# tl32rodan/DCVC

Hardware: AMD Instinct MI355X
Metric: encode+decode fps @1920x1080 per GPU; bpp bit-exact + PSNR Δ<1e-4 dB vs ref (higher is better)
Workload: dtype f32 (convs on split-fp16 f16x3 MFMA, fp32 accumulation); 1 GPU; C3 DCVC-DC RGB 1920x1080 (pad 1920x1088) IP=32 write mode; gop=32, precision=split, q_index=0, stream_part=8, parallelism=sequence-sharded x1, 3 GOP lane(s) per GPU, lanes=3, step=one frame on each of 3 lane(s)

## Files before the change

dcvc_amd/csrc/hip/sdc.hip:

```cpp
#include "common.h"
#include "split.h"

namespace {

constexpr int kNW = 8, kNT = kNW * 64;
constexpr int TH = 8, TW = 16;
constexpr int HW_ = TW + 2, NPH = (TH + 2) * HW_;
constexpr int HR = 192;

struct DP {
  const float *x;
  int H, W, xcs, xco;
  float *y;
  int ycs, yco;
  const uint16_t *w;
  int wbytes;
  const float *b1, *wdw, *bdw, *b2, *ba;
  float slope;
  int tiles_x, ntiles;
  int *ovf;
};

template <int CIN, int COUT, bool ADAPT>
struct DG {
  static constexpr int KCI = (CIN + 31) / 32;
  static constexpr int NTI = (CIN + 15) / 16, NTO = (COUT + 15) / 16;
  static constexpr int CI16 = NTI * 16, CO16 = NTO * 16;
  static constexpr int W1 = KCI * CI16 * 32, W2 = KCI * CO16 * 32, WA = ADAPT ? KCI * CO16 * 32 : 0;
  static constexpr int NWH = 2 * (W1 + W2 + WA);
  static constexpr int XI = KCI * HR * 32;
  static constexpr int DI = KCI * TH * TW * 32;
  static constexpr size_t OX = 0, OD = OX + (size_t)2 * XI * 2, OW = OD + (size_t)2 * DI * 2;
  static constexpr size_t OC = OW + (size_t)NWH * 2;
  static constexpr int NC = CIN * 11 + 2 * COUT;
  static constexpr size_t LDS = OC + (size_t)NC * 4;
  static constexpr int QP = CIN / 8;
  static constexpr int PP = (NPH * QP + kNT - 1) / kNT;
};

__device__ __forceinline__ float lrelu(float v, float s) { return fmaxf(v, v * s); }

template <int CIN, int COUT, bool ADAPT>
__global__ void __launch_bounds__(kNT) sdc_kernel(DP p) {
  SplitRange rg(p.ovf);
  typedef DG<CIN, COUT, ADAPT> G_;
  constexpr int KCI = G_::KCI, NTI = G_::NTI, NTO = G_::NTO, CO16 = G_::CO16, CI16 = G_::CI16;
  constexpr int XI = G_::XI, DI = G_::DI, QP = G_::QP, PP = G_::PP;
  extern __shared__ __align__(16) unsigned char smem[];
  uint16_t *Xh = reinterpret_cast<uint16_t *>(smem + G_::OX), *Xl = Xh + XI;
  uint16_t *Dh = reinterpret_cast<uint16_t *>(smem + G_::OD), *Dl = Dh + DI;
  uint16_t *W1h = reinterpret_cast<uint16_t *>(smem + G_::OW), *W1l = W1h + G_::W1;
  uint16_t *W2h = W1l + G_::W1, *W2l = W2h + G_::W2;
  uint16_t *WAh = W2l + G_::W2, *WAl = WAh + G_::WA;
  float *Lb1 = reinterpret_cast<float *>(smem + G_::OC), *Lbdw = Lb1 + CIN, *Lwdw = Lbdw + CIN;
  float *Lb2 = Lwdw + 9 * CIN, *Lba = Lb2 + COUT;
  auto t1p = [&](int r, int c) -> float * {
    return reinterpret_cast<float *>((c & 16) ? Xl : Xh) + (((c >> 5) * HR + r) * 16 + (c & 15));
  };

  const int tid = threadIdx.x;
  const int wave = tid >> 6, lane = tid & 63;
  const int col = lane & 15, hi = lane >> 4;
  const int G = gridDim.x;
  int g = blockIdx.x;
  if ((G & 7) == 0) g = (g & 7) * (G >> 3) + (g >> 3);
  if (g >= p.ntiles) return;

  {
    const __amdgpu_buffer_rsrc_t wr =
        __builtin_amdgcn_make_buffer_rsrc(const_cast<uint16_t *>(p.w), (short)0, p.wbytes, 0x00020000);
    constexpr int ND = G_::NWH * 2 / 1024;
    for (int i = wave; i < ND; i += kNW)
      __builtin_amdgcn_raw_ptr_buffer_load_lds(wr, (__attribute__((address_space(3))) void *)(W1h + i * 512), 16,
                                               i * 1024 + lane * 16, 0, 0, 0);
    for (int i = tid; i < G_::NC; i += kNT) {
      float v;
      if (i < CIN) v = p.b1[i];
      else if (i < 2 * CIN) v = p.bdw[i - CIN];
      else if (i < 11 * CIN) v = p.wdw[i - 2 * CIN];
      else if (i < 11 * CIN + COUT) v = p.b2[i - 11 * CIN];
      else v = ADAPT ? p.ba[i - 11 * CIN - COUT] : 0.f;
      Lb1[i] = v;
    }
  }

  const __amdgpu_buffer_rsrc_t xr = __builtin_amdgcn_make_buffer_rsrc(
      const_cast<float *>(p.x), (short)0,
      (int)((int64_t)p.H * p.W * p.xcs * 4 < 0x7fff0000 ? (int64_t)p.H * p.W * p.xcs * 4 : 0x7fff0000), 0x00020000);
  int pyx[PP], prel[PP], pofs[PP];
#pragma unroll
  for (int u = 0; u < PP; ++u) {
    const int it = tid + u * kNT;
    pyx[u] = -1;
    prel[u] = 0;
    pofs[u] = 0;
    if (it < NPH * QP) {
      const int pix = it / QP, q = it - pix * QP;
      const int hy = pix / HW_, hx = pix - hy * HW_;
      pyx[u] = (hy << 8) | hx;
      prel[u] = ((hy - 1) * p.W + (hx - 1)) * p.xcs + p.xco + q * 8;
      pofs[u] = swz((q >> 2) * HR + pix, q & 3);
    }
  }
  float pf[PP][8];
  auto prefetch = [&](int t) {
    const int oy0 = (t / p.tiles_x) * TH, ox0 = (t % p.tiles_x) * TW;
    const int base = oy0 * p.W + ox0;
#pragma unroll
    for (int u = 0; u < PP; ++u) {
      const int gy = oy0 - 1 + (pyx[u] >> 8), gx = ox0 - 1 + (pyx[u] & 255);
      const bool in = pyx[u] >= 0 && (unsigned)gy < (unsigned)p.H && (unsigned)gx < (unsigned)p.W;
      const int o = in ? (base * p.xcs + prel[u]) * 4 : 0x7fffffe0;
      const f32x4 a = __builtin_bit_cast(f32x4, __builtin_amdgcn_raw_buffer_load_b128(xr, o, 0, 0));
      const f32x4 b = __builtin_bit_cast(f32x4, __builtin_amdgcn_raw_buffer_load_b128(xr, o + 16, 0, 0));
#pragma unroll
      for (int j = 0; j < 4; ++j) {
        pf[u][j] = a[j];
        pf[u][4 + j] = b[j];
      }
    }
  };
  prefetch(g);

  auto zero_pad = [&]() {
    if constexpr (CIN % 32 != 0) {
      constexpr int PADQ = KCI * 4 - QP;
      for (int it = tid; it < HR * PADQ; it += kNT) {
        const int row = it / PADQ, q = QP + it % PADQ;
        const int o = swz((q >> 2) * HR + row, q & 3);
        *reinterpret_cast<u32x4_t *>(Xh + o) = u32x4_t{0u, 0u, 0u, 0u};
        *reinterpret_cast<u32x4_t *>(Xl + o) = u32x4_t{0u, 0u, 0u, 0u};
      }
    }
  };

  wait_vm_lgkm();
  for (int t = g; t < p.ntiles; t += G) {
    const int oy0 = (t / p.tiles_x) * TH, ox0 = (t % p.tiles_x) * TW;
    raw_barrier();
#pragma unroll
    for (int u = 0; u < PP; ++u) {
      u32x4_t h, l;
      rg.add8(pf[u]);
      split8(pf[u], h, l);
      if (pyx[u] >= 0) {
        *reinterpret_cast<u32x4_t *>(Xh + pofs[u]) = h;
        *reinterpret_cast<u32x4_t *>(Xl + pofs[u]) = l;
      }
    }
    zero_pad();
    wait_lgkm();
    raw_barrier();
    if (t + G < p.ntiles) prefetch(t + G);

    f32x4 idn[NTO];
    if constexpr (ADAPT) {
      f32x4 am[NTO], ac[NTO];
#pragma unroll
      for (int j = 0; j < NTO; ++j) {
        am[j] = f32x4{0.f, 0.f, 0.f, 0.f};
        ac[j] = f32x4{0.f, 0.f, 0.f, 0.f};
      }
      const int hr = (wave + 1) * HW_ + 1 + col;
#pragma unroll
      for (int kc = 0; kc < KCI; ++kc) {
        const int ob = swz(kc * HR + hr, hi);
        const f16x8 bh = *reinterpret_cast<const f16x8 *>(Xh + ob), bl = *reinterpret_cast<const f16x8 *>(Xl + ob);
#pragma unroll
        for (int j = 0; j < NTO; ++j) {
          const int oa = swz(kc * CO16 + j * 16 + col, hi);
          const f16x8 ah = *reinterpret_cast<const f16x8 *>(WAh + oa), al = *reinterpret_cast<const f16x8 *>(WAl + oa);
          am[j] = __builtin_amdgcn_mfma_f32_16x16x32_f16(ah, bh, am[j], 0, 0, 0);
          ac[j] = __builtin_amdgcn_mfma_f32_16x16x32_f16(ah, bl, ac[j], 0, 0, 0);
          ac[j] = __builtin_amdgcn_mfma_f32_16x16x32_f16(al, bh, ac[j], 0, 0, 0);
        }
      }
#pragma unroll
      for (int j = 0; j < NTO; ++j) {
        const int n = j * 16 + hi * 4;
#pragma unroll
        for (int e = 0; e < 4; ++e) idn[j][e] = (am[j][e] + ac[j][e] * kLoInv) + Lba[n + e < COUT ? n + e : 0];
      }
      wait_lgkm();
      raw_barrier();
    }

    for (int ht = wave; ht < HR / 16; ht += kNW) {
      f32x4 tm[NTI], tc[NTI];
#pragma unroll
      for (int j = 0; j < NTI; ++j) {
        tm[j] = f32x4{0.f, 0.f, 0.f, 0.f};
        tc[j] = f32x4{0.f, 0.f, 0.f, 0.f};
      }
      const int r = ht * 16 + col;
#pragma unroll
      for (int kc = 0; kc < KCI; ++kc) {
        const int ob = swz(kc * HR + r, hi);
        const f16x8 bh = *reinterpret_cast<const f16x8 *>(Xh + ob), bl = *reinterpret_cast<const f16x8 *>(Xl + ob);
#pragma unroll
        for (int j = 0; j < NTI; ++j) {
          const int oa = swz(kc * CI16 + j * 16 + col, hi);
          const f16x8 ah = *reinterpret_cast<const f16x8 *>(W1h + oa), al = *reinterpret_cast<const f16x8 *>(W1l + oa);
          tm[j] = __builtin_amdgcn_mfma_f32_16x16x32_f16(ah, bh, tm[j], 0, 0, 0);
          tc[j] = __builtin_amdgcn_mfma_f32_16x16x32_f16(ah, bl, tc[j], 0, 0, 0);
          tc[j] = __builtin_amdgcn_mfma_f32_16x16x32_f16(al, bh, tc[j], 0, 0, 0);
        }
      }
      const int hy = r / HW_, hx = r - hy * HW_;
      const int gy = oy0 - 1 + hy, gx = ox0 - 1 + hx;
      const bool inside = r < NPH && (unsigned)gy < (unsigned)p.H && (unsigned)gx < (unsigned)p.W;
      wave_lds_sync();
#pragma unroll
      for (int j = 0; j < NTI; ++j) {
        const int n = j * 16 + hi * 4;
        if (n >= CIN) continue;
        f32x4 v;
#pragma unroll
        for (int e = 0; e < 4; ++e) v[e] = inside ? lrelu((tm[j][e] + tc[j][e] * kLoInv) + Lb1[n + e], p.slope) : 0.f;
        *reinterpret_cast<f32x4 *>(t1p(r, n)) = v;
      }
    }
    wait_lgkm();
    raw_barrier();

    {
      constexpr int CG = CIN / 4;
      constexpr int R = kNT / (CG * TW) >= 4 ? 4 : kNT / (CG * TW) >= 2 ? 2 : 1;
      constexpr int RR = TH / R;
      static_assert(CG * TW * R <= kNT && TH % R == 0, "P2 tasks");
      if (tid < CG * TW * R) {
        const int cg = tid % CG, rest = tid / CG;
        const int ix = rest % TW, y0 = (rest / TW) * RR;
        const int c = cg * 4;
        f32x4 wv[9];
#pragma unroll
        for (int k = 0; k < 9; ++k) wv[k] = *reinterpret_cast<const f32x4 *>(Lwdw + k * CIN + c);
        const float4 bd = *reinterpret_cast<const float4 *>(Lbdw + c);
        f32x4 win[3][3];
#pragma unroll
        for (int r = 0; r < 2; ++r)
#pragma unroll
          for (int dx = 0; dx < 3; ++dx)
            win[r][dx] = *reinterpret_cast<const f32x4 *>(t1p((y0 + r) * HW_ + ix + dx, c));
#pragma unroll
        for (int i = 0; i < RR; ++i) {
#pragma unroll
          for (int dx = 0; dx < 3; ++dx)
            win[(i + 2) % 3][dx] = *reinterpret_cast<const f32x4 *>(t1p((y0 + i + 2) * HW_ + ix + dx, c));
          f32x4 a = f32x4{0.f, 0.f, 0.f, 0.f};
#pragma unroll
          for (int dy = 0; dy < 3; ++dy)
#pragma unroll
            for (int dx = 0; dx < 3; ++dx)
#pragma unroll
              for (int e = 0; e < 4; ++e) a[e] = __builtin_fmaf(wv[dy * 3 + dx][e], win[(i + dy) % 3][dx][e], a[e]);
          float v[4];
          v[0] = a[0] + bd.x;
          v[1] = a[1] + bd.y;
          v[2] = a[2] + bd.z;
          v[3] = a[3] + bd.w;
          rg.add4(v);
          const auto h01 = __builtin_amdgcn_cvt_pkrtz(v[0], v[1]);
          const auto h23 = __builtin_amdgcn_cvt_pkrtz(v[2], v[3]);
          const uint32_t l01 = pk(split_lo(v[0], (float)h01[0]), split_lo(v[1], (float)h01[1]));
          const uint32_t l23 = pk(split_lo(v[2], (float)h23[0]), split_lo(v[3], (float)h23[1]));
          const int px = (y0 + i) * TW + ix;
          const int o = swz((c >> 5) * (TH * TW) + px, (c & 31) >> 3) + (c & 7);
          typedef unsigned int u32x2_t __attribute__((ext_vector_type(2)));
          *reinterpret_cast<u32x2_t *>(Dh + o) = u32x2_t{__builtin_bit_cast(uint32_t, h01), __builtin_bit_cast(uint32_t, h23)};
          *reinterpret_cast<u32x2_t *>(Dl + o) = u32x2_t{l01, l23};
        }
      }
      if constexpr (CIN % 32 != 0) {
        constexpr int PADQ = KCI * 4 - CIN / 8;
        for (int it = tid; it < TH * TW * PADQ; it += kNT) {
          const int px = it / PADQ, q = CIN / 8 + it % PADQ;
          const int o = swz((q >> 2) * (TH * TW) + px, q & 3);
          *reinterpret_cast<u32x4_t *>(Dh + o) = u32x4_t{0u, 0u, 0u, 0u};
          *reinterpret_cast<u32x4_t *>(Dl + o) = u32x4_t{0u, 0u, 0u, 0u};
        }
      }
    }
    wait_lgkm();
    raw_barrier();

    {
      f32x4 cm[NTO], cc[NTO];
#pragma unroll
      for (int j = 0; j < NTO; ++j) {
        cm[j] = f32x4{0.f, 0.f, 0.f, 0.f};
        cc[j] = f32x4{0.f, 0.f, 0.f, 0.f};
      }
#pragma unroll
      for (int kc = 0; kc < KCI; ++kc) {
        const int ob = swz(kc * (TH * TW) + wave * TW + col, hi);
        const f16x8 bh = *reinterpret_cast<const f16x8 *>(Dh + ob), bl = *reinterpret_cast<const f16x8 *>(Dl + ob);
#pragma unroll
        for (int j = 0; j < NTO; ++j) {
          const int oa = swz(kc * CO16 + j * 16 + col, hi);
          const f16x8 ah = *reinterpret_cast<const f16x8 *>(W2h + oa), al = *reinterpret_cast<const f16x8 *>(W2l + oa);
          cm[j] = __builtin_amdgcn_mfma_f32_16x16x32_f16(ah, bh, cm[j], 0, 0, 0);
          cc[j] = __builtin_amdgcn_mfma_f32_16x16x32_f16(ah, bl, cc[j], 0, 0, 0);
          cc[j] = __builtin_amdgcn_mfma_f32_16x16x32_f16(al, bh, cc[j], 0, 0, 0);
        }
      }
      const int gy = oy0 + wave, gx = ox0 + col;
      if (gy < p.H && gx < p.W) {
        const int64_t pix = (int64_t)gy * p.W + gx;
#pragma unroll
        for (int j = 0; j < NTO; ++j) {
          const int n = j * 16 + hi * 4;
          if (n >= COUT) continue;
          f32x4 id;
          if constexpr (ADAPT) id = idn[j];
          else id = *reinterpret_cast<const f32x4 *>(p.x + pix * p.xcs + p.xco + n);
          f32x4 v;
#pragma unroll
          for (int e = 0; e < 4; ++e) v[e] = ((cm[j][e] + cc[j][e] * kLoInv) + Lb2[n + e]) + id[e];
          *reinterpret_cast<f32x4 *>(p.y + pix * p.ycs + p.yco + n) = v;
        }
      }
    }
  }
  wait_vm_lgkm();
}

int g_cus = 0;

template <int CIN, int COUT, bool ADAPT>
int run(DP p, hipStream_t st) {
  typedef DG<CIN, COUT, ADAPT> G_;
  static_assert(G_::LDS <= 160 * 1024, "LDS");
  static_assert(G_::NWH * 2 % 1024 == 0, "weight images in whole 1-KiB pieces");
  p.tiles_x = (p.W + TW - 1) / TW;
  const int64_t nt = (int64_t)p.tiles_x * ((p.H + TH - 1) / TH);
  if (nt <= 0) return DCVC_HIP_OK;
  p.ntiles = (int)nt;
  if (g_cus <= 0) {
    int dev = 0;
    hipDeviceProp_t prop;
    if (hipGetDevice(&dev) != hipSuccess || hipGetDeviceProperties(&prop, dev) != hipSuccess) return DCVC_HIP_ELAUNCH;
    g_cus = prop.multiProcessorCount;
  }
  int G = g_cus;
  if (G > p.ntiles) G = p.ntiles;
  auto kern = sdc_kernel<CIN, COUT, ADAPT>;
  dcvc_note_kernel("sdc_kernel<%d, %d, %s>@%lld", CIN, COUT, bname(ADAPT), (long long)G * kNT);
  dcvc_ensure_lds(reinterpret_cast<const void *>(kern), (int)G_::LDS);
  hipLaunchKernelGGL(kern, dim3((unsigned)G), dim3(kNT), G_::LDS, st, p);
  DCVC_LAUNCH_CHECK();
  return DCVC_HIP_OK;
}

bool supported(int cin, int cout, bool adapt) {
  return (cin == 64 && cout == 48 && adapt) || (cin == 48 && cout == 32 && adapt) ||
         (cin == 64 && cout == 64 && !adapt) || (cin == 32 && cout == 64 && adapt) ||
         (cin == 48 && cout == 48 && !adapt) || (cin == 32 && cout == 32 && !adapt);
}

}

extern "C" int64_t dcvc_dc_pack_weights(const float *w1, const float *w2, const float *wa, int cin, int cout,
                                        void *out) {
  if (!w1 || !w2 || cin <= 0 || cout <= 0) return DCVC_HIP_EINVAL;
  if (out && (!host_split_range_ok(w1, (int64_t)cin * cin) || !host_split_range_ok(w2, (int64_t)cout * cin) ||
              (wa && !host_split_range_ok(wa, (int64_t)cout * cin))))
    return DCVC_HIP_EINVAL;
  const int kci = (cin + 31) / 32, ci16 = (cin + 15) / 16 * 16, co16 = (cout + 15) / 16 * 16;
  const int64_t n1 = (int64_t)kci * ci16 * 32, n2 = (int64_t)kci * co16 * 32, na = wa ? n2 : 0;
  const int64_t total = 2 * (n1 + n2 + na);
  if (!out) return total;
  uint16_t *o = reinterpret_cast<uint16_t *>(out);
  auto at = [](int row, int k) {
    const int x = (0x1320 >> (((row >> 2) & 3) << 2)) & 3;
    return (int64_t)row * 32 + ((((k >> 3) ^ x) & 3) << 3) + (k & 7);
  };
  auto put = [&](uint16_t *img, int64_t n, const float *w, int rows, int rows16) {
    for (int kc = 0; kc < kci; ++kc)
      for (int r = 0; r < rows16; ++r)
        for (int k = 0; k < 32; ++k) {
          const int ch = kc * 32 + k;
          const float v = (r < rows && ch < cin) ? w[(int64_t)r * cin + ch] : 0.f;
          const int64_t q = at(kc * rows16 + r, k);
          host_split(v, img[q], img[n + q]);
        }
  };
  put(o, n1, w1, cin, ci16);
  put(o + 2 * n1, n2, w2, cout, co16);
  if (wa) put(o + 2 * n1 + 2 * n2, na, wa, cout, co16);
  return total;
}

extern "C" int dcvc_depth_conv_split(const dcvc_dc_args *a, void *stream) {
  if (!a || !a->x.ptr || !a->y.ptr || !a->w || !a->b1 || !a->wdw || !a->bdw || !a->b2) return DCVC_HIP_EINVAL;
  if (a->x.dtype != DCVC_F32 || a->y.dtype != DCVC_F32 || a->x.C != a->cin || a->y.C != a->cout ||
      a->x.H != a->y.H || a->x.W != a->y.W)
    return DCVC_HIP_EINVAL;
  const bool adapt = a->adaptor != 0;
  if (!supported(a->cin, a->cout, adapt) || (adapt && !a->ba)) return DCVC_HIP_EUNSUPPORTED;
  if (!(a->slope >= 0.f && a->slope <= 1.f)) return DCVC_HIP_EUNSUPPORTED;
  if (a->x.cstride % 4 || a->x.coff % 4 || a->y.cstride % 4 || a->y.coff % 4 || ((uintptr_t)a->x.ptr & 15) ||
      ((uintptr_t)a->y.ptr & 15))
    return DCVC_HIP_EUNSUPPORTED;
  if ((int64_t)a->x.H * a->x.W * a->x.cstride * 4 >= 0x7fff0000) return DCVC_HIP_EUNSUPPORTED;
  DP p{};
  p.ovf = dcvc_internal_split_flag();
  p.x = reinterpret_cast<const float *>(a->x.ptr);
  p.H = a->x.H;
  p.W = a->x.W;
  p.xcs = a->x.cstride;
  p.xco = a->x.coff;
  p.y = reinterpret_cast<float *>(a->y.ptr);
  p.ycs = a->y.cstride;
  p.yco = a->y.coff;
  p.w = reinterpret_cast<const uint16_t *>(a->w);
  p.wbytes = (int)(dcvc_dc_pack_weights(reinterpret_cast<const float *>(1), reinterpret_cast<const float *>(1),
                                        adapt ? reinterpret_cast<const float *>(1) : nullptr, a->cin, a->cout,
                                        nullptr) * 2);
  p.b1 = a->b1;
  p.wdw = a->wdw;
  p.bdw = a->bdw;
  p.b2 = a->b2;
  p.ba = a->ba;
  p.slope = a->slope;
  hipStream_t st = reinterpret_cast<hipStream_t>(stream);
  if (a->cin == 64 && a->cout == 48) return run<64, 48, true>(p, st);
  if (a->cin == 48 && a->cout == 32) return run<48, 32, true>(p, st);
  if (a->cin == 32 && a->cout == 64) return run<32, 64, true>(p, st);
  if (a->cin == 64 && a->cout == 64) return run<64, 64, false>(p, st);
  if (a->cin == 48 && a->cout == 48) return run<48, 48, false>(p, st);
  return run<32, 32, false>(p, st);
}
```

dcvc_amd/hip.py:

```python
import ctypes
import os
import threading

import numpy as np
import torch

from ._native import NativeError, hip_lib, check

F32, BF16 = 0, 1
F16X3 = 2
ACT_NONE, ACT_LRELU, ACT_CLAMP01, ACT_ROUND = 0, 1, 2, 3
IN_NONE, IN_LRELU, IN_GATE = 0, 1, 2

_TORCH = {F32: torch.float32, BF16: torch.bfloat16}
_CNAME = {F32: "f32", BF16: "bf16", F16X3: "f16x3"}
_CODE = {torch.float32: F32, torch.bfloat16: BF16}


class CTensor(ctypes.Structure):
    _fields_ = [("ptr", ctypes.c_void_p), ("dtype", ctypes.c_int), ("H", ctypes.c_int),
                ("W", ctypes.c_int), ("C", ctypes.c_int), ("cstride", ctypes.c_int),
                ("coff", ctypes.c_int)]


# ... 18 lines not shown
                ("res", CTensor), ("res2", CTensor)]


class CFfnArgs(ctypes.Structure):
    _fields_ = [("x", CTensor), ("y", CTensor), ("c", ctypes.c_int), ("hidden", ctypes.c_int),
                ("w", ctypes.c_void_p), ("b1", ctypes.c_void_p), ("b2", ctypes.c_void_p),
                ("scale", ctypes.c_void_p), ("slope", ctypes.c_float)]


class CDcArgs(ctypes.Structure):
    _fields_ = [("x", CTensor), ("y", CTensor), ("cin", ctypes.c_int), ("cout", ctypes.c_int),
                ("adaptor", ctypes.c_int), ("w", ctypes.c_void_p), ("b1", ctypes.c_void_p), ("wdw", ctypes.c_void_p),
                ("bdw", ctypes.c_void_p), ("b2", ctypes.c_void_p), ("ba", ctypes.c_void_p), ("slope", ctypes.c_float)]


class CDwcArgs(ctypes.Structure):
    _fields_ = [("t", CTensor), ("r", CTensor), ("y", CTensor), ("c", ctypes.c_int), ("w9", ctypes.c_void_p),
                ("bdw", ctypes.c_void_p), ("w2", ctypes.c_void_p), ("b2", ctypes.c_void_p)]


_T = CTensor
_vp, _i, _f = ctypes.c_void_p, ctypes.c_int, ctypes.c_float
HIP_SYMBOLS = [
    ("dcvc_conv_pack_weights", ctypes.c_int64, [_vp, _i, _i, _i, _i, _i, _vp]),
    ("dcvc_conv2d", _i, [ctypes.POINTER(CConvArgs), _vp]),
    ("dcvc_set_option", _i, [ctypes.c_char_p, _i]),
    ("dcvc_split_range_flag", _i, [_vp]),
    ("dcvc_last_kernel", ctypes.c_char_p, []),
    ("dcvc_depthconv_block", _i, [ctypes.POINTER(CDcbArgs), _vp]),
    ("dcvc_ffn_pack_weights", ctypes.c_int64, [_vp, _vp, _i, _i, _vp]),
    ("dcvc_conv_ffn", _i, [ctypes.POINTER(CFfnArgs), _vp]),
    ("dcvc_dc_pack_weights", ctypes.c_int64, [_vp, _vp, _vp, _i, _i, _vp]),
    ("dcvc_depth_conv_split", _i, [ctypes.POINTER(CDcArgs), _vp]),
    ("dcvc_frag_pack_weights", ctypes.c_int64, [_vp, _i, _i, _vp]),
    ("dcvc_dw_conv2_split", _i, [ctypes.POINTER(CDwcArgs), _vp]),
    ("dcvc_dwconv3x3", _i, [_T, _T, _vp, _vp, _vp]),
    ("dcvc_flow_warp", _i, [_T, _T, _T, _vp, _vp, _vp]),
    ("dcvc_offset_diversity", _i, [_T, _T, _T, _T, _vp, _vp, _vp, _vp, _f, _vp]),
    ("dcvc_offset_diversity_workspace", ctypes.c_int64, [_i, _i]),
    ("dcvc_offset_diversity_ws", _i, [_T, _T, _T, _T, _vp, _vp, _vp, _vp, _f, _vp, ctypes.c_int64, _vp]),
    ("dcvc_resize2x", _i, [_T, _T, _i, _f, _vp]),
    ("dcvc_pool2x2", _i, [_T, _T, _i, _vp]),
    ("dcvc_add", _i, [_T, _T, _T, _vp]),
    ("dcvc_copy", _i, [_T, _T, _vp]),
    ("dcvc_pad_replicate", _i, [_T, _T, _vp]),
    ("dcvc_frame_to_nhwc", _i, [_vp, _i, _i, _T, _vp]),
    ("dcvc_frame_to_nhwc_zero_pad", _i, [_vp, _i, _i, _T, _vp]),
    ("dcvc_yuv420_to_nhwc", _i, [_vp, _vp, _i, _i, _T, _vp]),
    ("dcvc_frame_sse_workspace", ctypes.c_int64, []),
    ("dcvc_frame_sse", _i, [_T, _vp, _vp, _i, _i, _i, _vp, _vp, _vp]),
    ("dcvc_recon_to_u8", _i, [_T, _i, _i, _i, _vp, _vp]),
    ("dcvc_quadtree_encode_step", _i, [_T, _T, _T, _i, _T, _T, _vp, _vp, _f, _f, _vp]),
    ("dcvc_quadtree_indexes_step", _i, [_T, _T, _i, _vp, _f, _f, _vp]),
    ("dcvc_quadtree_decode_step", _i, [_T, _T, _i, _vp, _T, _T, _vp]),
    ("dcvc_nhwc_to_symbols", _i, [_T, _vp, _vp]),
    ("dcvc_symbols_to_nhwc", _i, [_vp, _T, _vp]),
    ("dcvc_quadtree_estimate_step", _i, [_T, _T, _T, _i, _T, _T, _vp, _i, _vp]),
    ("dcvc_factorized_bits", _i, [_T, _vp, _vp, _vp]),
    ("dcvc_sum_f32", _i, [_vp, ctypes.c_int64, _vp, _vp]),
    ("dcvc_dual_prior_encode_step", _i, [_T, _T, _T, _i, _T, _vp, _vp, _vp, _f, _f, _vp]),
    ("dcvc_dual_prior_indexes_step", _i, [_T, _T, _i, _vp, _f, _f, _vp]),
    ("dcvc_dual_prior_decode_step", _i, [_T, _T, _i, _vp, _T, _vp, _vp]),
    ("dcvc_dual_prior_estimate_step", _i, [_T, _T, _T, _i, _T, _vp, _vp, _i, _f, _vp]),
    ("dcvc_channel_div", _i, [_T, _vp, _T, _vp]),
    ("dcvc_fill", _i, [_T, _f, _vp]),
    ("dcvc_nhwc_to_symbols_i32", _i, [_T, _vp, _vp]),
# ... 685 lines not shown
```

include/dcvc_hip.h:

```cpp
#ifndef DCVC_HIP_H
#define DCVC_HIP_H

#include <stdint.h>

#ifdef __cplusplus
extern "C" {
#endif

#define DCVC_HIP_OK 0
#define DCVC_HIP_EINVAL (-1)
#define DCVC_HIP_ELAUNCH (-2)
#define DCVC_HIP_EUNSUPPORTED (-3)

enum dcvc_dtype { DCVC_F32 = 0, DCVC_BF16 = 1 };
#define DCVC_F16X3 2

enum dcvc_act {
  DCVC_ACT_NONE = 0,
  DCVC_ACT_LRELU = 1,
  DCVC_ACT_CLAMP01 = 2,
  DCVC_ACT_ROUND = 3
};

enum dcvc_in_op {
// ... 49 lines not shown
} dcvc_dcb_args;
int dcvc_depthconv_block(const dcvc_dcb_args *a, void *stream);

typedef struct dcvc_ffn_args {
  dcvc_tensor x, y;
  int c, hidden;
  const void *w;
  const float *b1, *b2;
  const float *scale;
  float slope;
} dcvc_ffn_args;
int64_t dcvc_ffn_pack_weights(const float *w1, const float *w2, int c, int hidden, void *out);
int dcvc_conv_ffn(const dcvc_ffn_args *a, void *stream);

typedef struct dcvc_dwc_args {
  dcvc_tensor t, r, y;
  int c;
  const float *w9, *bdw;
  const void *w2;
  const float *b2;
} dcvc_dwc_args;
int64_t dcvc_frag_pack_weights(const float *w, int rows, int k, void *out);
int dcvc_dw_conv2_split(const dcvc_dwc_args *a, void *stream);

typedef struct dcvc_dc_args {
  dcvc_tensor x, y;
  int cin, cout, adaptor;
  const void *w;
  const float *b1, *wdw, *bdw, *b2, *ba;
  float slope;
} dcvc_dc_args;
int64_t dcvc_dc_pack_weights(const float *w1, const float *w2, const float *wa, int cin, int cout, void *out);
int dcvc_depth_conv_split(const dcvc_dc_args *a, void *stream);

int dcvc_dwconv3x3(dcvc_tensor x, dcvc_tensor y, const float *w,
                   const float *bias, void *stream);

int dcvc_flow_warp(dcvc_tensor x, dcvc_tensor flow, dcvc_tensor y,
                   const float *gx, const float *gy, void *stream);

int dcvc_offset_diversity(dcvc_tensor feat, dcvc_tensor offs_half,
                          dcvc_tensor flow, dcvc_tensor y, const float *fw,
                          const float *fb, const float *gx, const float *gy,
                          float max_mag, void *stream);

int64_t dcvc_offset_diversity_workspace(int H, int W);
int dcvc_offset_diversity_ws(dcvc_tensor feat, dcvc_tensor offs_half,
                             dcvc_tensor flow, dcvc_tensor y, const float *fw,
                             const float *fb, const float *gx, const float *gy,
                             float max_mag, void *workspace, int64_t ws_bytes,
                             void *stream);

int dcvc_resize2x(dcvc_tensor x, dcvc_tensor y, int up, float mul,
                  void *stream);
int dcvc_pool2x2(dcvc_tensor x, dcvc_tensor y, int is_max, void *stream);

int dcvc_add(dcvc_tensor a, dcvc_tensor b, dcvc_tensor y, void *stream);
int dcvc_copy(dcvc_tensor x, dcvc_tensor y, void *stream);
int dcvc_pad_replicate(dcvc_tensor x, dcvc_tensor y, void *stream);
int dcvc_frame_to_nhwc(const uint8_t *src, int h, int w, dcvc_tensor y,
                       void *stream);
int dcvc_frame_to_nhwc_zero_pad(const uint8_t *src, int h, int w, dcvc_tensor y,
                                void *stream);
int dcvc_yuv420_to_nhwc(const uint8_t *y, const uint8_t *uv, int h, int w,
                        dcvc_tensor out, void *stream);
int64_t dcvc_frame_sse_workspace(void);
// ... 73 lines not shown
```

Baseline: 30.39 frames/s.

## Rewrite depth-conv block as per-wave vertical strip streaming with register windows

```diff
diff --git a/dcvc_amd/csrc/hip/sdc.hip b/dcvc_amd/csrc/hip/sdc.hip
--- a/dcvc_amd/csrc/hip/sdc.hip
+++ b/dcvc_amd/csrc/hip/sdc.hip
@@ -1,12 +1,9 @@
 #include "common.h"
 #include "split.h"
 
+#include <type_traits>
+
 namespace {
-
-constexpr int kNW = 8, kNT = kNW * 64;
-constexpr int TH = 8, TW = 16;
-constexpr int HW_ = TW + 2, NPH = (TH + 2) * HW_;
-constexpr int HR = 192;
 
 struct DP {
   const float *x;
@@ -17,7 +14,7 @@
   int wbytes;
   const float *b1, *wdw, *bdw, *b2, *ba;
   float slope;
-  int tiles_x, ntiles;
+  int sh, strips, nitems;
   int *ovf;
 };
 
@@ -28,43 +25,67 @@
   static constexpr int CI16 = NTI * 16, CO16 = NTO * 16;
   static constexpr int W1 = KCI * CI16 * 32, W2 = KCI * CO16 * 32, WA = ADAPT ? KCI * CO16 * 32 : 0;
   static constexpr int NWH = 2 * (W1 + W2 + WA);
-  static constexpr int XI = KCI * HR * 32;
-  static constexpr int DI = KCI * TH * TW * 32;
-  static constexpr size_t OX = 0, OD = OX + (size_t)2 * XI * 2, OW = OD + (size_t)2 * DI * 2;
-  static constexpr size_t OC = OW + (size_t)NWH * 2;
   static constexpr int NC = CIN * 11 + 2 * COUT;
-  static constexpr size_t LDS = OC + (size_t)NC * 4;
-  static constexpr int QP = CIN / 8;
-  static constexpr int PP = (NPH * QP + kNT - 1) / kNT;
 };
 
 __device__ __forceinline__ float lrelu(float v, float s) { return fmaxf(v, v * s); }
 
+constexpr int SW = 14;
+constexpr int kSegMin = 4;
+constexpr int kSegMax = 128;
+
 template <int CIN, int COUT, bool ADAPT>
-__global__ void __launch_bounds__(kNT) sdc_kernel(DP p) {
+struct SG {
+  typedef DG<CIN, COUT, ADAPT> D_;
+  static constexpr size_t OC = (size_t)D_::NWH * 2;
+  static constexpr size_t LDS = OC + (size_t)D_::NC * 4;
+  static_assert(CIN % 16 == 0 && COUT % 16 == 0, "whole 16-channel tiles");
+};
+
+template <int CTRL>
+__device__ __forceinline__ f32x4 row_shift(const f32x4 &v) {
+  f32x4 r = v;
+#ifdef __HIP_DEVICE_COMPILE__
+#pragma unroll
+  for (int e = 0; e < 4; ++e)
+    r[e] = __int_as_float(__builtin_amdgcn_update_dpp(0, __float_as_int(v[e]), CTRL, 0xf, 0xf, true));
+#endif
+  return r;
+}
+constexpr int kRowShr1 = 0x111, kRowShl1 = 0x101;
+
+__device__ __forceinline__ void relay2(uint32_t a, uint32_t b, uint32_t &d0, uint32_t &d2) {
+#ifdef __HIP_DEVICE_COMPILE__
+  const auto s = __builtin_amdgcn_permlane32_swap(a, b, false, false);
+  const auto t = __builtin_amdgcn_permlane16_swap(s[0], s[1], false, false);
+  d0 = t[0];
+  d2 = t[1];
+#else
+  d0 = a;
+  d2 = b;
+#endif
+}
+
+template <int CIN, int COUT, bool ADAPT, int NW>
+__global__ void __launch_bounds__(NW * 64) __attribute__((amdgpu_waves_per_eu(NW / 4, NW / 4))) sdc_kernel_strip(DP p) {
+  constexpr int kNW = NW, kNT = NW * 64;
   SplitRange rg(p.ovf);
   typedef DG<CIN, COUT, ADAPT> G_;
+  typedef SG<CIN, COUT, ADAPT> S_;
   constexpr int KCI = G_::KCI, NTI = G_::NTI, NTO = G_::NTO, CO16 = G_::CO16, CI16 = G_::CI16;
-  constexpr int XI = G_::XI, DI = G_::DI, QP = G_::QP, PP = G_::PP;
   extern __shared__ __align__(16) unsigned char smem[];
-  uint16_t *Xh = reinterpret_cast<uint16_t *>(smem + G_::OX), *Xl = Xh + XI;
-  uint16_t *Dh = reinterpret_cast<uint16_t *>(smem + G_::OD), *Dl = Dh + DI;
-  uint16_t *W1h = reinterpret_cast<uint16_t *>(smem + G_::OW), *W1l = W1h + G_::W1;
+  uint16_t *W1h = reinterpret_cast<uint16_t *>(smem), *W1l = W1h + G_::W1;
   uint16_t *W2h = W1l + G_::W1, *W2l = W2h + G_::W2;
   uint16_t *WAh = W2l + G_::W2, *WAl = WAh + G_::WA;
-  float *Lb1 = reinterpret_cast<float *>(smem + G_::OC), *Lbdw = Lb1 + CIN, *Lwdw = Lbdw + CIN;
+  float *Lb1 = reinterpret_cast<float *>(smem + S_::OC), *Lbdw = Lb1 + CIN, *Lwdw = Lbdw + CIN;
   float *Lb2 = Lwdw + 9 * CIN, *Lba = Lb2 + COUT;
-  auto t1p = [&](int r, int c) -> float * {
-    return reinterpret_cast<float *>((c & 16) ? Xl : Xh) + (((c >> 5) * HR + r) * 16 + (c & 15));
-  };
 
   const int tid = threadIdx.x;
-  const int wave = tid >> 6, lane = tid & 63;
+  const int wave = __builtin_amdgcn_readfirstlane(tid >> 6), lane = tid & 63;
   const int col = lane & 15, hi = lane >> 4;
   const int G = gridDim.x;
   int g = blockIdx.x;
   if ((G & 7) == 0) g = (g & 7) * (G >> 3) + (g >> 3);
-  if (g >= p.ntiles) return;
 
   {
     const __amdgpu_buffer_rsrc_t wr =
@@ -83,208 +104,140 @@
       Lb1[i] = v;
     }
   }
+  wait_vm_lgkm();
+  __syncthreads();
 
   const __amdgpu_buffer_rsrc_t xr = __builtin_amdgcn_make_buffer_rsrc(
       const_cast<float *>(p.x), (short)0,
       (int)((int64_t)p.H * p.W * p.xcs * 4 < 0x7fff0000 ? (int64_t)p.H * p.W * p.xcs * 4 : 0x7fff0000), 0x00020000);
-  int pyx[PP], prel[PP], pofs[PP];
-#pragma unroll
-  for (int u = 0; u < PP; ++u) {
-    const int it = tid + u * kNT;
-    pyx[u] = -1;
-    prel[u] = 0;
-    pofs[u] = 0;
-    if (it < NPH * QP) {
-      const int pix = it / QP, q = it - pix * QP;
-      const int hy = pix / HW_, hx = pix - hy * HW_;
-      pyx[u] = (hy << 8) | hx;
-      prel[u] = ((hy - 1) * p.W + (hx - 1)) * p.xcs + p.xco + q * 8;
-      pofs[u] = swz((q >> 2) * HR + pix, q & 3);
-    }
-  }
-  float pf[PP][8];
-  auto prefetch = [&](int t) {
-    const int oy0 = (t / p.tiles_x) * TH, ox0 = (t % p.tiles_x) * TW;
-    const int base = oy0 * p.W + ox0;
-#pragma unroll
-    for (int u = 0; u < PP; ++u) {
-      const int gy = oy0 - 1 + (pyx[u] >> 8), gx = ox0 - 1 + (pyx[u] & 255);
-      const bool in = pyx[u] >= 0 && (unsigned)gy < (unsigned)p.H && (unsigned)gx < (unsigned)p.W;
-      const int o = in ? (base * p.xcs + prel[u]) * 4 : 0x7fffffe0;
-      const f32x4 a = __builtin_bit_cast(f32x4, __builtin_amdgcn_raw_buffer_load_b128(xr, o, 0, 0));
-      const f32x4 b = __builtin_bit_cast(f32x4, __builtin_amdgcn_raw_buffer_load_b128(xr, o + 16, 0, 0));
-#pragma unroll
-      for (int j = 0; j < 4; ++j) {
-        pf[u][j] = a[j];
-        pf[u][4 + j] = b[j];
-      }
-    }
-  };
-  prefetch(g);
-
-  auto zero_pad = [&]() {
-    if constexpr (CIN % 32 != 0) {
-      constexpr int PADQ = KCI * 4 - QP;
-      for (int it = tid; it < HR * PADQ; it += kNT) {
-        const int row = it / PADQ, q = QP + it % PADQ;
-        const int o = swz((q >> 2) * HR + row, q & 3);
-        *reinterpret_cast<u32x4_t *>(Xh + o) = u32x4_t{0u, 0u, 0u, 0u};
-        *reinterpret_cast<u32x4_t *>(Xl + o) = u32x4_t{0u, 0u, 0u, 0u};
-      }
-    }
-  };
-
-  wait_vm_lgkm();
-  for (int t = g; t < p.ntiles; t += G) {
-    const int oy0 = (t / p.tiles_x) * TH, ox0 = (t % p.tiles_x) * TW;
-    raw_barrier();
-#pragma unroll
-    for (int u = 0; u < PP; ++u) {
-      u32x4_t h, l;
-      rg.add8(pf[u]);
-      split8(pf[u], h, l);
-      if (pyx[u] >= 0) {
-        *reinterpret_cast<u32x4_t *>(Xh + pofs[u]) = h;
-        *reinterpret_cast<u32x4_t *>(Xl + pofs[u]) = l;
-      }
-    }
-    zero_pad();
-    wait_lgkm();
-    raw_barrier();
-    if (t + G < p.ntiles) prefetch(t + G);
-
-    f32x4 idn[NTO];
-    if constexpr (ADAPT) {
-      f32x4 am[NTO], ac[NTO];
-#pragma unroll
-      for (int j = 0; j < NTO; ++j) {
-        am[j] = f32x4{0.f, 0.f, 0.f, 0.f};
-        ac[j] = f32x4{0.f, 0.f, 0.f, 0.f};
-      }
-      const int hr = (wave + 1) * HW_ + 1 + col;
+  const __amdgpu_buffer_rsrc_t yr = __builtin_amdgcn_make_buffer_rsrc(
+      p.y, (short)0, (int)((int64_t)p.H * p.W * p.ycs * 4), 0x00020000);
+  const int aw = swz(col, hi);
+
+  for (int it = wave * G + g; it < p.nitems; it += G * kNW) {
+    const int seg = it / p.strips, strip = it - seg * p.strips;
+    const int y0 = seg * p.sh, x0 = strip * SW;
+    const int ye = y0 + p.sh < p.H ? y0 + p.sh : p.H;
+    const int gx = x0 - 1 + col;
+    const bool xin = (unsigned)gx < (unsigned)p.W;
+    const bool ok = xin && col >= 1 && col <= SW;
+    uint32_t okm = ok ? 0xffffffffu : 0u;
+    opaque_v(okm);
+    auto ofs = [&](int o) { return (int)(((uint32_t)o & okm) | (0x7fffffe0u & ~okm)); };
+
+    float pf[KCI][8];
+    auto load_row = [&](int gy) {
+      const bool in = xin && (unsigned)gy < (unsigned)p.H && gy <= ye;
 #pragma unroll
       for (int kc = 0; kc < KCI; ++kc) {
-        const int ob = swz(kc * HR + hr, hi);
-        const f16x8 bh = *reinterpret_cast<const f16x8 *>(Xh + ob), bl = *reinterpret_cast<const f16x8 *>(Xl + ob);
-#pragma unroll
-        for (int j = 0; j < NTO; ++j) {
-          const int oa = swz(kc * CO16 + j * 16 + col, hi);
-          const f16x8 ah = *reinterpret_cast<const f16x8 *>(WAh + oa), al = *reinterpret_cast<const f16x8 *>(WAl + oa);
-          am[j] = __builtin_amdgcn_mfma_f32_16x16x32_f16(ah, bh, am[j], 0, 0, 0);
-          ac[j] = __builtin_amdgcn_mfma_f32_16x16x32_f16(ah, bl, ac[j], 0, 0, 0);
-          ac[j] = __builtin_amdgcn_mfma_f32_16x16x32_f16(al, bh, ac[j], 0, 0, 0);
-        }
-      }
-#pragma unroll
-      for (int j = 0; j < NTO; ++j) {
-        const int n = j * 16 + hi * 4;
-#pragma unroll
-        for (int e = 0; e < 4; ++e) idn[j][e] = (am[j][e] + ac[j][e] * kLoInv) + Lba[n + e < COUT ? n + e : 0];
-      }
-      wait_lgkm();
-      raw_barrier();
-    }
-
-    for (int ht = wave; ht < HR / 16; ht += kNW) {
-      f32x4 tm[NTI], tc[NTI];
-#pragma unroll
-      for (int j = 0; j < NTI; ++j) {
-        tm[j] = f32x4{0.f, 0.f, 0.f, 0.f};
-        tc[j] = f32x4{0.f, 0.f, 0.f, 0.f};
-      }
-      const int r = ht * 16 + col;
+        const int ch = kc * 32 + hi * 8;
+        const int o = (in && ch < CIN) ? ((gy * p.W + gx) * p.xcs + p.xco + ch) * 4 : 0x7fffffe0;
+        const f32x4 a = __builtin_bit_cast(f32x4, __builtin_amdgcn_raw_buffer_load_b128(xr, o, 0, 0));
+        const f32x4 b = __builtin_bit_cast(f32x4, __builtin_amdgcn_raw_buffer_load_b128(xr, o + 16, 0, 0));
+#pragma unroll
+        for (int e = 0; e < 4; ++e) {
+          pf[kc][e] = a[e];
+          pf[kc][4 + e] = b[e];
+        }
+      }
+    };
+
+    f32x4 win[3][NTI];
+    f16x8 xh[KCI], xl[KCI];
+    auto step = [&](auto Sc, auto Ec, int gy) {
+      constexpr int S = decltype(Sc)::value;
+      constexpr bool emit = decltype(Ec)::value;
+      f32x4 am[NTO], ac[NTO], idx[NTO];
+      if constexpr (emit) {
+        if constexpr (ADAPT) {
+#pragma unroll
+          for (int j = 0; j < NTO; ++j) {
+            am[j] = f32x4{0.f, 0.f, 0.f, 0.f};
+            ac[j] = f32x4{0.f, 0.f, 0.f, 0.f};
+          }
+#pragma unroll
+          for (int kc = 0; kc < KCI; ++kc)
+#pragma unroll
+            for (int j = 0; j < NTO; ++j) {
+              const int oa = aw + (kc * CO16 + j * 16) * 32;
+              const f16x8 ah = *reinterpret_cast<const f16x8 *>(WAh + oa), al = *reinterpret_cast<const f16x8 *>(WAl + oa);
+              am[j] = __builtin_amdgcn_mfma_f32_16x16x32_f16(ah, xh[kc], am[j], 0, 0, 0);
+              ac[j] = __builtin_amdgcn_mfma_f32_16x16x32_f16(ah, xl[kc], ac[j], 0, 0, 0);
+              ac[j] = __builtin_amdgcn_mfma_f32_16x16x32_f16(al, xh[kc], ac[j], 0, 0, 0);
+            }
+        } else {
+          const int xo = ofs((((gy - 1) * p.W + gx) * p.xcs + p.xco + hi * 4) * 4);
+#pragma unroll
+          for (int j = 0; j < NTO; ++j)
+            idx[j] = __builtin_bit_cast(f32x4, __builtin_amdgcn_raw_buffer_load_b128(xr, xo, j * 64, 0));
+        }
+      }
 #pragma unroll
       for (int kc = 0; kc < KCI; ++kc) {
-        const int ob = swz(kc * HR + r, hi);
-        const f16x8 bh = *reinterpret_cast<const f16x8 *>(Xh + ob), bl = *reinterpret_cast<const f16x8 *>(Xl + ob);
+        u32x4_t h, l;
+        rg.add8(pf[kc]);
+        split8(pf[kc], h, l);
+        xh[kc] = __builtin_bit_cast(f16x8, h);
+        xl[kc] = __builtin_bit_cast(f16x8, l);
+      }
+      load_row(gy + 1);
+      {
+        f32x4 tm[NTI], tc[NTI];
 #pragma unroll
         for (int j = 0; j < NTI; ++j) {
-          const int oa = swz(kc * CI16 + j * 16 + col, hi);
-          const f16x8 ah = *reinterpret_cast<const f16x8 *>(W1h + oa), al = *reinterpret_cast<const f16x8 *>(W1l + oa);
-          tm[j] = __builtin_amdgcn_mfma_f32_16x16x32_f16(ah, bh, tm[j], 0, 0, 0);
-          tc[j] = __builtin_amdgcn_mfma_f32_16x16x32_f16(ah, bl, tc[j], 0, 0, 0);
-          tc[j] = __builtin_amdgcn_mfma_f32_16x16x32_f16(al, bh, tc[j], 0, 0, 0);
-        }
-      }
-      const int hy = r / HW_, hx = r - hy * HW_;
-      const int gy = oy0 - 1 + hy, gx = ox0 - 1 + hx;
-      const bool inside = r < NPH && (unsigned)gy < (unsigned)p.H && (unsigned)gx < (unsigned)p.W;
-      wave_lds_sync();
+          tm[j] = f32x4{0.f, 0.f, 0.f, 0.f};
+          tc[j] = f32x4{0.f, 0.f, 0.f, 0.f};
+        }
+#pragma unroll
+        for (int kc = 0; kc < KCI; ++kc)
+#pragma unroll
+          for (int j = 0; j < NTI; ++j) {
+            const int oa = aw + (kc * CI16 + j * 16) * 32;
+            const f16x8 ah = *reinterpret_cast<const f16x8 *>(W1h + oa), al = *reinterpret_cast<const f16x8 *>(W1l + oa);
+            tm[j] = __builtin_amdgcn_mfma_f32_16x16x32_f16(ah, xh[kc], tm[j], 0, 0, 0);
+            tc[j] = __builtin_amdgcn_mfma_f32_16x16x32_f16(ah, xl[kc], tc[j], 0, 0, 0);
+            tc[j] = __builtin_amdgcn_mfma_f32_16x16x32_f16(al, xh[kc], tc[j], 0, 0, 0);
+          }
+        const uint32_t inm = (xin && (unsigned)gy < (unsigned)p.H) ? 0xffffffffu : 0u;
+#pragma unroll
+        for (int j = 0; j < NTI; ++j) {
+          const f32x4 b = *reinterpret_cast<const f32x4 *>(Lb1 + j * 16 + hi * 4);
+#pragma unroll
+          for (int e = 0; e < 4; ++e)
+            win[S][j][e] = __uint_as_float(__float_as_uint(lrelu((tm[j][e] + tc[j][e] * kLoInv) + b[e], p.slope)) & inm);
+        }
+      }
+      if constexpr (!emit) return;
+      uint32_t dh[NTI][2], dl[NTI][2];
 #pragma unroll
       for (int j = 0; j < NTI; ++j) {
         const int n = j * 16 + hi * 4;
-        if (n >= CIN) continue;
-        f32x4 v;
-#pragma unroll
-        for (int e = 0; e < 4; ++e) v[e] = inside ? lrelu((tm[j][e] + tc[j][e] * kLoInv) + Lb1[n + e], p.slope) : 0.f;
-        *reinterpret_cast<f32x4 *>(t1p(r, n)) = v;
-      }
-    }
-    wait_lgkm();
-    raw_barrier();
-
-    {
-      constexpr int CG = CIN / 4;
-      constexpr int R = kNT / (CG * TW) >= 4 ? 4 : kNT / (CG * TW) >= 2 ? 2 : 1;
-      constexpr int RR = TH / R;
-      static_assert(CG * TW * R <= kNT && TH % R == 0, "P2 tasks");
-      if (tid < CG * TW * R) {
-        const int cg = tid % CG, rest = tid / CG;
-        const int ix = rest % TW, y0 = (rest / TW) * RR;
-        const int c = cg * 4;
-        f32x4 wv[9];
-#pragma unroll
-        for (int k = 0; k < 9; ++k) wv[k] = *reinterpret_cast<const f32x4 *>(Lwdw + k * CIN + c);
-        const float4 bd = *reinterpret_cast<const float4 *>(Lbdw + c);
-        f32x4 win[3][3];
-#pragma unroll
-        for (int r = 0; r < 2; ++r)
-#pragma unroll
-          for (int dx = 0; dx < 3; ++dx)
-            win[r][dx] = *reinterpret_cast<const f32x4 *>(t1p((y0 + r) * HW_ + ix + dx, c));
-#pragma unroll
-        for (int i = 0; i < RR; ++i) {
-#pragma unroll
-          for (int dx = 0; dx < 3; ++dx)
-            win[(i + 2) % 3][dx] = *reinterpret_cast<const f32x4 *>(t1p((y0 + i + 2) * HW_ + ix + dx, c));
-          f32x4 a = f32x4{0.f, 0.f, 0.f, 0.f};
-#pragma unroll
-          for (int dy = 0; dy < 3; ++dy)
-#pragma unroll
-            for (int dx = 0; dx < 3; ++dx)
-#pragma unroll
-              for (int e = 0; e < 4; ++e) a[e] = __builtin_fmaf(wv[dy * 3 + dx][e], win[(i + dy) % 3][dx][e], a[e]);
-          float v[4];
-          v[0] = a[0] + bd.x;
-          v[1] = a[1] + bd.y;
-          v[2] = a[2] + bd.z;
-          v[3] = a[3] + bd.w;
-          rg.add4(v);
-          const auto h01 = __builtin_amdgcn_cvt_pkrtz(v[0], v[1]);
-          const auto h23 = __builtin_amdgcn_cvt_pkrtz(v[2], v[3]);
-          const uint32_t l01 = pk(split_lo(v[0], (float)h01[0]), split_lo(v[1], (float)h01[1]));
-          const uint32_t l23 = pk(split_lo(v[2], (float)h23[0]), split_lo(v[3], (float)h23[1]));
-          const int px = (y0 + i) * TW + ix;
-          const int o = swz((c >> 5) * (TH * TW) + px, (c & 31) >> 3) + (c & 7);
-          typedef unsigned int u32x2_t __attribute__((ext_vector_type(2)));
-          *reinterpret_cast<u32x2_t *>(Dh + o) = u32x2_t{__builtin_bit_cast(uint32_t, h01), __builtin_bit_cast(uint32_t, h23)};
-          *reinterpret_cast<u32x2_t *>(Dl + o) = u32x2_t{l01, l23};
-        }
-      }
-      if constexpr (CIN % 32 != 0) {
-        constexpr int PADQ = KCI * 4 - CIN / 8;
-        for (int it = tid; it < TH * TW * PADQ; it += kNT) {
-          const int px = it / PADQ, q = CIN / 8 + it % PADQ;
-          const int o = swz((q >> 2) * (TH * TW) + px, q & 3);
-          *reinterpret_cast<u32x4_t *>(Dh + o) = u32x4_t{0u, 0u, 0u, 0u};
-          *reinterpret_cast<u32x4_t *>(Dl + o) = u32x4_t{0u, 0u, 0u, 0u};
-        }
-      }
-    }
-    wait_lgkm();
-    raw_barrier();
-
-    {
+        f32x4 a = f32x4{0.f, 0.f, 0.f, 0.f};
+#pragma unroll
+        for (int dy = 0; dy < 3; ++dy) {
+          const f32x4 &c = win[(S + 1 + dy) % 3][j];
+          const f32x4 t[3] = {row_shift<kRowShr1>(c), c, row_shift<kRowShl1>(c)};
+#pragma unroll
+          for (int dx = 0; dx < 3; ++dx) {
+            const f32x4 w = *reinterpret_cast<const f32x4 *>(Lwdw + (dy * 3 + dx) * CIN + n);
+#pragma unroll
+            for (int e = 0; e < 4; ++e) a[e] = __builtin_fmaf(w[e], t[dx][e], a[e]);
+          }
+        }
+        const f32x4 bd = *reinterpret_cast<const f32x4 *>(Lbdw + n);
+        float v[4];
+#pragma unroll
+        for (int e = 0; e < 4; ++e) v[e] = a[e] + bd[e];
+        const uint32_t m0 = rg.m;
+        rg.add4(v);
+        rg.m = max(m0, rg.m & okm);
+        const auto h01 = __builtin_amdgcn_cvt_pkrtz(v[0], v[1]);
+        const auto h23 = __builtin_amdgcn_cvt_pkrtz(v[2], v[3]);
+        dh[j][0] = __builtin_bit_cast(uint32_t, h01);
+        dh[j][1] = __builtin_bit_cast(uint32_t, h23);
+        dl[j][0] = pk(split_lo(v[0], (float)h01[0]), split_lo(v[1], (float)h01[1]));
+        dl[j][1] = pk(split_lo(v[2], (float)h23[0]), split_lo(v[3], (float)h23[1]));
+      }
       f32x4 cm[NTO], cc[NTO];
 #pragma unroll
       for (int j = 0; j < NTO; ++j) {
@@ -293,61 +246,112 @@
       }
 #pragma unroll
       for (int kc = 0; kc < KCI; ++kc) {
-        const int ob = swz(kc * (TH * TW) + wave * TW + col, hi);
-        const f16x8 bh = *reinterpret_cast<const f16x8 *>(Dh + ob), bl = *reinterpret_cast<const f16x8 *>(Dl + ob);
+        uint32_t bh[4], bl[4];
+        constexpr uint32_t Z = 0u;
+        const bool two = 2 * kc + 1 < NTI;
+        const int ja = 2 * kc, jb = two ? 2 * kc + 1 : 2 * kc;
+        relay2(dh[ja][0], two ? dh[jb][0] : Z, bh[0], bh[2]);
+        relay2(dh[ja][1], two ? dh[jb][1] : Z, bh[1], bh[3]);
+        relay2(dl[ja][0], two ? dl[jb][0] : Z, bl[0], bl[2]);
+        relay2(dl[ja][1], two ? dl[jb][1] : Z, bl[1], bl[3]);
+        const f16x8 vh = __builtin_bit_cast(f16x8, u32x4_t{bh[0], bh[1], bh[2], bh[3]});
+        const f16x8 vl = __builtin_bit_cast(f16x8, u32x4_t{bl[0], bl[1], bl[2], bl[3]});
 #pragma unroll
         for (int j = 0; j < NTO; ++j) {
-          const int oa = swz(kc * CO16 + j * 16 + col, hi);
+          const int oa = aw + (kc * CO16 + j * 16) * 32;
           const f16x8 ah = *reinterpret_cast<const f16x8 *>(W2h + oa), al = *reinterpret_cast<const f16x8 *>(W2l + oa);
-          cm[j] = __builtin_amdgcn_mfma_f32_16x16x32_f16(ah, bh, cm[j], 0, 0, 0);
-          cc[j] = __builtin_amdgcn_mfma_f32_16x16x32_f16(ah, bl, cc[j], 0, 0, 0);
-          cc[j] = __builtin_amdgcn_mfma_f32_16x16x32_f16(al, bh, cc[j], 0, 0, 0);
-        }
-      }
-      const int gy = oy0 + wave, gx = ox0 + col;
-      if (gy < p.H && gx < p.W) {
-        const int64_t pix = (int64_t)gy * p.W + gx;
+          cm[j] = __builtin_amdgcn_mfma_f32_16x16x32_f16(ah, vh, cm[j], 0, 0, 0);
+          cc[j] = __builtin_amdgcn_mfma_f32_16x16x32_f16(ah, vl, cc[j], 0, 0, 0);
+          cc[j] = __builtin_amdgcn_mfma_f32_16x16x32_f16(al, vh, cc[j], 0, 0, 0);
+        }
+      }
+      {
+        const int yo = ofs((((gy - 1) * p.W + gx) * p.ycs + p.yco + hi * 4) * 4);
 #pragma unroll
         for (int j = 0; j < NTO; ++j) {
           const int n = j * 16 + hi * 4;
-          if (n >= COUT) continue;
+          const f32x4 b2 = *reinterpret_cast<const f32x4 *>(Lb2 + n);
           f32x4 id;
-          if constexpr (ADAPT) id = idn[j];
-          else id = *reinterpret_cast<const f32x4 *>(p.x + pix * p.xcs + p.xco + n);
+          if constexpr (ADAPT) {
+            const f32x4 ba = *reinterpret_cast<const f32x4 *>(Lba + n);
+#pragma unroll
+            for (int e = 0; e < 4; ++e) id[e] = (am[j][e] + ac[j][e] * kLoInv) + ba[e];
+          } else {
+            id = idx[j];
+          }
           f32x4 v;
 #pragma unroll
-          for (int e = 0; e < 4; ++e) v[e] = ((cm[j][e] + cc[j][e] * kLoInv) + Lb2[n + e]) + id[e];
-          *reinterpret_cast<f32x4 *>(p.y + pix * p.ycs + p.yco + n) = v;
-        }
-      }
+          for (int e = 0; e < 4; ++e) v[e] = ((cm[j][e] + cc[j][e] * kLoInv) + b2[e]) + id[e];
+          __builtin_amdgcn_raw_buffer_store_b128(__builtin_bit_cast(u32x4_t, v), yr, yo, j * 64, 0);
+        }
+      }
+    };
+
+    int gy = y0 - 1;
+    load_row(gy);
+    step(std::integral_constant<int, 0>{}, std::false_type{}, gy++);
+    step(std::integral_constant<int, 1>{}, std::false_type{}, gy++);
+#pragma unroll 1
+    for (;;) {
+      step(std::integral_constant<int, 2>{}, std::true_type{}, gy);
+      if (++gy > ye) break;
+      step(std::integral_constant<int, 0>{}, std::true_type{}, gy);
+      if (++gy > ye) break;
+      step(std::integral_constant<int, 1>{}, std::true_type{}, gy);
+      if (++gy > ye) break;
     }
   }
-  wait_vm_lgkm();
 }
 
 int g_cus = 0;
 
-template <int CIN, int COUT, bool ADAPT>
-int run(DP p, hipStream_t st) {
-  typedef DG<CIN, COUT, ADAPT> G_;
-  static_assert(G_::LDS <= 160 * 1024, "LDS");
-  static_assert(G_::NWH * 2 % 1024 == 0, "weight images in whole 1-KiB pieces");
-  p.tiles_x = (p.W + TW - 1) / TW;
-  const int64_t nt = (int64_t)p.tiles_x * ((p.H + TH - 1) / TH);
-  if (nt <= 0) return DCVC_HIP_OK;
-  p.ntiles = (int)nt;
+int cus() {
   if (g_cus <= 0) {
     int dev = 0;
     hipDeviceProp_t prop;
-    if (hipGetDevice(&dev) != hipSuccess || hipGetDeviceProperties(&prop, dev) != hipSuccess) return DCVC_HIP_ELAUNCH;
+    if (hipGetDevice(&dev) != hipSuccess || hipGetDeviceProperties(&prop, dev) != hipSuccess) return 0;
     g_cus = prop.multiProcessorCount;
   }
-  int G = g_cus;
-  if (G > p.ntiles) G = p.ntiles;
-  auto kern = sdc_kernel<CIN, COUT, ADAPT>;
-  dcvc_note_kernel("sdc_kernel<%d, %d, %s>@%lld", CIN, COUT, bname(ADAPT), (long long)G * kNT);
-  dcvc_ensure_lds(reinterpret_cast<const void *>(kern), (int)G_::LDS);
-  hipLaunchKernelGGL(kern, dim3((unsigned)G), dim3(kNT), G_::LDS, st, p);
+  return g_cus;
+}
+
+constexpr int waves_of(int cin, int cout) { return (cin == cout && cin >= 48) ? 8 : 12; }
+
+int seg_rows(int H, int W, int ncu, int kNW) {
+  const int strips = (W + SW - 1) / SW;
+  const int64_t nwaves = (int64_t)ncu * kNW;
+  int best = kSegMin;
+  int64_t bc = INT64_MAX;
+  for (int sh = kSegMin; sh <= kSegMax; ++sh) {
+    const int64_t items = (int64_t)strips * ((H + sh - 1) / sh);
+    const int64_t cost = ((items + nwaves - 1) / nwaves) * ((sh < H ? sh : H) + 2);
+    if (cost < bc) {
+      bc = cost;
+      best = sh;
+    }
+  }
+  return best;
+}
+
+template <int CIN, int COUT, bool ADAPT, int NW>
+int run_strip(DP p, hipStream_t st) {
+  constexpr int kNW = NW, kNT = NW * 64;
+  typedef SG<CIN, COUT, ADAPT> S_;
+  static_assert(S_::LDS <= 160 * 1024, "LDS");
+  static_assert(S_::D_::NWH * 2 % 1024 == 0, "weight images in whole 1-KiB pieces");
+  if (p.H <= 0 || p.W <= 0) return DCVC_HIP_OK;
+  const int ncu = cus();
+  if (ncu <= 0) return DCVC_HIP_ELAUNCH;
+  p.sh = seg_rows(p.H, p.W, ncu, NW);
+  p.strips = (p.W + SW - 1) / SW;
+  const int64_t ni = (int64_t)p.strips * ((p.H + p.sh - 1) / p.sh);
+  if (ni >= ((int64_t)1 << 31) - ncu * kNW) return DCVC_HIP_EUNSUPPORTED;
+  p.nitems = (int)ni;
+  const int G = p.nitems < ncu ? p.nitems : ncu;
+  auto kern = sdc_kernel_strip<CIN, COUT, ADAPT, NW>;
+  dcvc_note_kernel("sdc_kernel_strip<%d, %d, %s, %d>@%lld", CIN, COUT, bname(ADAPT), NW, (long long)G * kNT);
+  dcvc_ensure_lds(reinterpret_cast<const void *>(kern), (int)S_::LDS);
+  hipLaunchKernelGGL(kern, dim3((unsigned)G), dim3(kNT), S_::LDS, st, p);
   DCVC_LAUNCH_CHECK();
   return DCVC_HIP_OK;
 }
@@ -391,6 +395,12 @@
   return total;
 }
 
+extern "C" int dcvc_dc_segment_rows(int cin, int cout, int H, int W) {
+  const int ncu = cus();
+  if (H <= 0 || W <= 0 || ncu <= 0) return DCVC_HIP_EINVAL;
+  return seg_rows(H, W, ncu, waves_of(cin, cout));
+}
+
 extern "C" int dcvc_depth_conv_split(const dcvc_dc_args *a, void *stream) {
   if (!a || !a->x.ptr || !a->y.ptr || !a->w || !a->b1 || !a->wdw || !a->bdw || !a->b2) return DCVC_HIP_EINVAL;
   if (a->x.dtype != DCVC_F32 || a->y.dtype != DCVC_F32 || a->x.C != a->cin || a->y.C != a->cout ||
@@ -403,6 +413,7 @@
       ((uintptr_t)a->y.ptr & 15))
     return DCVC_HIP_EUNSUPPORTED;
   if ((int64_t)a->x.H * a->x.W * a->x.cstride * 4 >= 0x7fff0000) return DCVC_HIP_EUNSUPPORTED;
+  if ((int64_t)a->y.H * a->y.W * a->y.cstride * 4 >= 0x7fff0000) return DCVC_HIP_EUNSUPPORTED;
   DP p{};
   p.ovf = dcvc_internal_split_flag();
   p.x = reinterpret_cast<const float *>(a->x.ptr);
@@ -424,10 +435,14 @@
   p.ba = a->ba;
   p.slope = a->slope;
   hipStream_t st = reinterpret_cast<hipStream_t>(stream);
-  if (a->cin == 64 && a->cout == 48) return run<64, 48, true>(p, st);
-  if (a->cin == 48 && a->cout == 32) return run<48, 32, true>(p, st);
-  if (a->cin == 32 && a->cout == 64) return run<32, 64, true>(p, st);
-  if (a->cin == 64 && a->cout == 64) return run<64, 64, false>(p, st);
-  if (a->cin == 48 && a->cout == 48) return run<48, 48, false>(p, st);
-  return run<32, 32, false>(p, st);
-}
+#define SDC_RUN(CI, CO, AD) \
+  if (a->cin == CI && a->cout == CO) return run_strip<CI, CO, AD, waves_of(CI, CO)>(p, st);
+  SDC_RUN(64, 48, true)
+  SDC_RUN(48, 32, true)
+  SDC_RUN(32, 64, true)
+  SDC_RUN(64, 64, false)
+  SDC_RUN(48, 48, false)
+  SDC_RUN(32, 32, false)
+#undef SDC_RUN
+  return DCVC_HIP_EUNSUPPORTED;
+}
diff --git a/dcvc_amd/hip.py b/dcvc_amd/hip.py
--- a/dcvc_amd/hip.py
+++ b/dcvc_amd/hip.py
@@ -74,6 +74,7 @@
     ("dcvc_conv_ffn", _i, [ctypes.POINTER(CFfnArgs), _vp]),
     ("dcvc_dc_pack_weights", ctypes.c_int64, [_vp, _vp, _vp, _i, _i, _vp]),
     ("dcvc_depth_conv_split", _i, [ctypes.POINTER(CDcArgs), _vp]),
+    ("dcvc_dc_segment_rows", _i, [_i, _i, _i, _i]),
     ("dcvc_frag_pack_weights", ctypes.c_int64, [_vp, _i, _i, _vp]),
     ("dcvc_dw_conv2_split", _i, [ctypes.POINTER(CDwcArgs), _vp]),
     ("dcvc_dwconv3x3", _i, [_T, _T, _vp, _vp, _vp]),
diff --git a/include/dcvc_hip.h b/include/dcvc_hip.h
--- a/include/dcvc_hip.h
+++ b/include/dcvc_hip.h
@@ -105,6 +105,7 @@
 } dcvc_dc_args;
 int64_t dcvc_dc_pack_weights(const float *w1, const float *w2, const float *wa, int cin, int cout, void *out);
 int dcvc_depth_conv_split(const dcvc_dc_args *a, void *stream);
+int dcvc_dc_segment_rows(int cin, int cout, int H, int W);
 
 int dcvc_dwconv3x3(dcvc_tensor x, dcvc_tensor y, const float *w,
                    const float *bias, void *stream);
```

Result: no change. 30.68 frames/s, median of 6 (+1.0%).
